# HandBrake/HandBrake

Measured on AMD Instinct MI355X. Metric: filtered frames/sec, 1080p YUV420p NLMeans+decomb chain, higher is better.
Workload: dtype u8 (f32 NLMeans weights, 16-bit fixed-point scaler as zimg, sharpen mix = the reference's f64 expression, as one f32 multiply where init proves that equal); 1 GPU; BASELINE configs[3]: decomb(31, EEDI2 bob) -> nlmeans medium -> cropscale lanczos 1920x1080 -> 3840x2160 -> lapsharp, 1080i YUV420P 8-bit in, inputs resident in HBM; input=1920x1080, output=3840x2160, streams_per_gpu=1, content=interlaced, stream_frames=48, stage_streams=2, parallelism=1 GPU(s) x 1 independent stream(s), device=AMD Radeon Graphics (gfx950:sramecc+:xnack-, 256 CUs)

## Files before the change

### handbrake_amd/csrc/eedi2.hip

```cpp
#include "eedi2_common.h"
#include "eedi2_vote.h"
#include "eedi2_dirmap_vote.h"
#include "eedi2_dense.h"
#include "eedi2_engine.h"
#include "eedi2_mask_cells.h"
#include "eedi2_corner.h"

#include <atomic>
#include <algorithm>

namespace {

constexpr int PEAK = 255, NEUTRAL = 128;
constexpr int EEDI_MAX_FIELDS = EEDI_MAX_BATCH;
constexpr size_t GUARD = 32768;

__constant__ uint8_t c_limlut[33] = { 6, 6, 7, 7, 8, 8, 9, 9, 9, 10, 10, 11, 11, 12, 12, 12, 12, 12, 12, 12,
                                      12, 12, 12, 12, 12, 12, 12, 12, 12, 12, 12, 255, 255 };

constexpr int LIM_N = 33, LIM_PAD = 40;
__device__ __forceinline__ void lim_fill(uint8_t *tab, int tid)
{
    if (tid < LIM_N) tab[tid] = c_limlut[tid];
}
// ... 377 lines not shown
        const uint8_t *mc = Q.a + (size_t)y * pitch;
        if (mc[x] == PEAK && (mc[x - 1] == PEAK || mc[x + 1] == PEAK))
            list[atomicAdd(count, 1)] = (uint32_t)x | ((uint32_t)y << 14) | ((uint32_t)pl << 28);
    }
}

__global__ __launch_bounds__(256) void k_calc_dir_work(P3 P, const uint32_t *__restrict__ list,
                                                       const int *__restrict__ count, int maxd, int nt13, int nt19)
{
    const int gid = blockIdx.x * blockDim.x + threadIdx.x;
    if (gid >= *count) return;
    const uint32_t e = list[gid];
    const int x = e & 0x3fff, y = (e >> 14) & 0x3fff, pl = e >> 28;
    const PL Q = plane_ptrs(P, pl, 0);
    const int pitch = P.pitch[pl], width = P.width[pl], height = P.height[pl];
    const uint8_t *mc = Q.a + (size_t)y * pitch;
    const uint8_t *mp = mc - pitch, *mn = mc + pitch;
    const uint8_t *sc = Q.b + (size_t)y * pitch;
    const uint8_t *sp = sc - pitch, *sn = sc + pitch, *s2p = sp - pitch, *s2n = sn + pitch;
    const int maxdt = pl == 0 ? maxd : (maxd >> 1);
    const int startu = max(-x + 1, -maxdt), stopu = min(width - 2 - x, maxdt);
    const int vert = iabs((int)sc[x] - (int)sn[x]) + iabs((int)sc[x] - (int)sp[x]);
    int minb = min(nt13, vert * 6), mina = min(nt19, vert * 9);
    int minc = mina, mind = minb, mine = minb;
    int dira = -5000, dirb = -5000, dirc = -5000, dird = -5000, dire = -5000;
    for (int u = startu; u <= stopu; u++)
    {
        if (!(y == 1 || mp[x - 1 + u] == PEAK || mp[x + u] == PEAK || mp[x + 1 + u] == PEAK)) continue;
        if (!(y == height - 2 || mn[x - 1 - u] == PEAK || mn[x - u] == PEAK || mn[x + 1 - u] == PEAK)) continue;
        const int diffsn = sad3(sc, x, sn, x - u);
        const int diffsp = sad3(sc, x, sp, x + u);
        const int diffps = sad3(sp, x, sc, x - u);
        const int diffns = sad3(sn, x, sc, x + u);
        const int diff = diffsn + diffsp + diffps + diffns;
        int diffd = diffsp + diffns, diffe = diffsn + diffps;
        if (diff < minb) { dirb = u; minb = diff; }
        if (y > 1)
        {
            const int diff2pp = sad3(s2p, x, sp, x - u);
            const int diffp2p = sad3(sp, x, s2p, x + u);
            const int diffa = diff + diff2pp + diffp2p;
            diffd += diffp2p;
            diffe += diff2pp;
            if (diffa < mina) { dira = u; mina = diffa; }
        }
        if (y < height - 2)
        {
            const int diff2nn = sad3(s2n, x, sn, x + u);
            const int diffn2n = sad3(sn, x, s2n, x - u);
            const int diffc = diff + diff2nn + diffn2n;
            diffd += diff2nn;
            diffe += diffn2n;
            if (diffc < minc) { dirc = u; minc = diffc; }
        }
        if (diffd < mind) { dird = u; mind = diffd; }
        if (diffe < mine) { dire = u; mine = diffe; }
    }
    int order[5], k = 0;
    if (dira != -5000) order[k++] = dira;
    if (dirb != -5000) order[k++] = dirb;
    if (dirc != -5000) order[k++] = dirc;
    if (dird != -5000) order[k++] = dird;
    if (dire != -5000) order[k++] = dire;
    int out = NEUTRAL;
    if (k > 1)
    {
        const int mid = sorted_mid(order, k);
        const int tlim = max((int)c_limlut[iabs(mid)] >> 2, 2);
        int sum = 0, cnt = 0;
        for (int i = 0; i < k; i++)
            if (iabs(order[i] - mid) <= tlim) { cnt++; sum += order[i]; }
        if (cnt > 1) out = (NEUTRAL + ((int)((float)sum / (float)cnt) * 4)) & 0xff;
    }
    Q.c[(size_t)y * pitch + x] = (uint8_t)out;
}

#ifdef HBHIP_DEV_STATS
__device__ unsigned long long g_cd_stats[24];
#define CD_STAT(i, v) atomicAdd(&g_cd_stats[i], (unsigned long long)(v))
#else
#define CD_STAT(i, v) ((void)0)
#endif
constexpr int CD_W = 256, CD_HALO = 32, CD_LW = CD_W + 2 * CD_HALO;



__device__ __forceinline__ int calc_dir_vote(int ta, int tb, int tc, int td, int te)
{
    constexpr int BIG = 1 << 20;
    int v0 = ta ? ta - 32 : BIG, v1 = tb ? tb - 32 : BIG, v2 = tc ? tc - 32 : BIG, v3 = td ? td - 32 : BIG, v4 = te ? te - 32 : BIG;
    const int k = (ta != 0) + (tb != 0) + (tc != 0) + (td != 0) + (te != 0);
#define CD_CX(a, b) { const int lo_ = min(a, b), hi_ = max(a, b); a = lo_; b = hi_; }
    CD_CX(v0, v1) CD_CX(v3, v4) CD_CX(v2, v4) CD_CX(v2, v3) CD_CX(v0, v3) CD_CX(v0, v2) CD_CX(v1, v4) CD_CX(v1, v3) CD_CX(v1, v2)
#undef CD_CX
    int out = NEUTRAL;
    if (k > 1)
    {
        const int lo = k == 2 ? v0 : (k == 5 ? v2 : v1);
        const int hi = k >= 4 ? v2 : v1;
        const int mid = (lo + hi + 1) >> 1;
        static_assert(CD_HALO - 2 <= 30, "the closed form of limlut covers entries 0..30");
        const int tlim = iabs(mid) >= 13 ? 3 : 2;
        int sum = 0, cnt = 0;
        if (iabs(v0 - mid) <= tlim) { cnt++; sum += v0; }
        if (iabs(v1 - mid) <= tlim) { cnt++; sum += v1; }
        if (iabs(v2 - mid) <= tlim) { cnt++; sum += v2; }
        if (iabs(v3 - mid) <= tlim) { cnt++; sum += v3; }
        if (iabs(v4 - mid) <= tlim) { cnt++; sum += v4; }
        if (cnt > 1) out = (NEUTRAL + ((int)((float)sum / (float)cnt) * 4)) & 0xff;
    }
    return out;
}

template <bool EDGE, typename PASS>
__device__ __forceinline__ int calc_dir_search(const uint32_t *tr, PASS pass, int maxdt, bool first, bool last, int nt13, int nt19)
{
    const uint32_t F2p = tr[0], Fp = tr[CD_LW], Fc = tr[2 * CD_LW], Fn = tr[3 * CD_LW], F2n = tr[4 * CD_LW];
    const int ctr = (int)((Fc >> 8) & 0xff);
    const int vert = iabs(ctr - (int)((Fn >> 8) & 0xff)) + iabs(ctr - (int)((Fp >> 8) & 0xff));
    uint32_t kb = (uint32_t)min(nt13, vert * 6) << 16, ka = (uint32_t)min(nt19, vert * 9) << 16;
    uint32_t kc = ka, kd = kb, ke = kb;
    typedef __attribute__((address_space(3))) const uint32_t *lds_u32;
    uint32_t ap0 = (uint32_t)(uintptr_t)(lds_u32)(tr - maxdt), am0 = (uint32_t)(uintptr_t)(lds_u32)(tr + maxdt);
    uint32_t tag0 = (uint32_t)(32 - maxdt);
    asm volatile("" : "+v"(ap0), "+v"(am0), "+s"(tag0));
#define SADH(a, b, acc) __builtin_amdgcn_sad_hi_u8((a), (b), (acc))
    while (pass)
    {
        const int jj = sizeof(PASS) == 8 ? __ffsll((unsigned long long)pass) - 1 : __ffs((unsigned int)pass) - 1;
        pass &= pass - (PASS)1;
        const uint32_t tag = (uint32_t)jj + tag0;
        const lds_u32 tp = (lds_u32)(uintptr_t)(ap0 + 4u * (uint32_t)jj), tm = (lds_u32)(uintptr_t)(am0 - 4u * (uint32_t)jj);
        const uint32_t e1 = SADH(Fp, tm[2 * CD_LW], SADH(Fc, tm[3 * CD_LW], 0u));
        const uint32_t d1 = SADH(Fn, tp[2 * CD_LW], SADH(Fc, tp[1 * CD_LW], tag));
        const uint32_t diff = e1 + d1;
        uint32_t diffd = d1, diffe = e1;
        kb = min(kb, diff);
        if (!EDGE || !first)
        {
            const uint32_t diff2pp = SADH(F2p, tm[1 * CD_LW], tag);
            const uint32_t diffp2p = SADH(Fp, tp[0 * CD_LW], 0u);
            diffd += diffp2p;
            diffe += diff2pp;
            ka = min(ka, diff + diff2pp + diffp2p);
        }
        else
            diffe += tag;
        if (!EDGE || !last)
        {
            const uint32_t diff2nn = SADH(F2n, tp[3 * CD_LW], 0u);
            const uint32_t diffn2n = SADH(Fn, tm[4 * CD_LW], 0u);
            diffd += diff2nn;
            diffe += diffn2n;
            kc = min(kc, diff + diff2nn + diffn2n);
        }
        kd = min(kd, diffd);
        ke = min(ke, diffe);
    }
#undef SADH
    return calc_dir_vote((int)((ka & 0xffffu) >> 1), (int)(kb & 0xffffu), (int)(kc & 0xffffu), (int)(kd & 0xffffu), (int)(ke & 0xffffu));
}

template <int R, bool PRED>
__device__ __forceinline__ void calc_dir_dense(const uint32_t *tr, int maxdt, const uint32_t (&up)[R], const uint32_t (&dn)[R],
                                               int nt13, int nt19, uint32_t (&ka)[R], uint32_t (&kb)[R], uint32_t (&kc)[R],
                                               uint32_t (&kd)[R], uint32_t (&ke)[R])
{
    constexpr int NS = R + 4, NE = R + 3;
#define SADH(a, b, acc) __builtin_amdgcn_sad_hi_u8((a), (b), (acc))
    uint32_t T[NS];
#pragma unroll
    for (int r = 0; r < NS; r++) T[r] = tr[r * CD_LW];
#pragma unroll
    for (int j = 0; j < R; j++)
    {
        const int ctr = (int)((T[j + 2] >> 8) & 0xff);
        const int vert = iabs(ctr - (int)((T[j + 3] >> 8) & 0xff)) + iabs(ctr - (int)((T[j + 1] >> 8) & 0xff));
        kb[j] = (uint32_t)min(nt13, vert * 6) << 16; ka[j] = (uint32_t)min(nt19, vert * 9) << 16;
        kc[j] = ka[j]; kd[j] = kb[j]; ke[j] = kb[j];
    }
    {
        CdRun<R, PRED> run;
#pragma unroll
        for (int r = 0; r < NE; r++)
        {
            const uint32_t Pv = SADH(T[r], T[r + 1], 32u);
            run.push(r, Pv, Pv);
            if (r >= 3)
            {
                const int j = r - 3;
                const uint32_t X = PRED ? (up[j] << 30) & 0x40000000u : 0u;
                uint32_t ca, cb, cc, cd, ce;
                run.cands(j, X, ca, cb, cc, cd, ce);
                ka[j] = min(ka[j], ca); kb[j] = min(kb[j], cb); kc[j] = min(kc[j], cc); kd[j] = min(kd[j], cd); ke[j] = min(ke[j], ce);
                CD_FENCE_KEYS(j);
            }
        }
    }
    for (int d = 1; d <= maxdt; d++)
    {
        const uint32_t *tp = tr + d, *tm = tr - d;
        const uint32_t t1 = 32u + (uint32_t)d, t2 = 32u - (uint32_t)d, sh = 30u - (uint32_t)d;
        CdRun<R, PRED> pos, neg;
        uint32_t Pl0 = tp[0], Mi0 = tm[0], Pl1 = tp[CD_LW], Mi1 = tm[CD_LW];
#pragma unroll
        for (int r = 0; r < NE; r++)
        {
            uint32_t Pl2 = 0, Mi2 = 0;
            if (r + 2 < NS) { Pl2 = tp[(r + 2) * CD_LW]; Mi2 = tm[(r + 2) * CD_LW]; }
            pos.push(r, SADH(T[r], Mi1, t1), SADH(Pl0, T[r + 1], t1));
            neg.push(r, SADH(T[r], Pl1, t2), SADH(Mi0, T[r + 1], t2));
            Pl0 = Pl1; Mi0 = Mi1; Pl1 = Pl2; Mi1 = Mi2;
            if (r >= 3)
            {
                const int j = r - 3;
                const uint32_t X1 = PRED ? (up[j] << sh) & 0x40000000u : 0u, X2 = PRED ? (dn[j] << sh) & 0x40000000u : 0u;
                uint32_t ca, cb, cc, cd, ce, na, nb, nc, nd, ne;
                pos.cands(j, X1, ca, cb, cc, cd, ce);
                neg.cands(j, X2, na, nb, nc, nd, ne);
                ka[j] = min(ka[j], min(ca, na)); kb[j] = min(kb[j], min(cb, nb)); kc[j] = min(kc[j], min(cc, nc));
                kd[j] = min(kd[j], min(cd, nd)); ke[j] = min(ke[j], min(ce, ne));
                CD_FENCE_KEYS(j);
            }
        }
    }
#undef SADH
}

template <int N, bool PRED, int RD, int J0>
__device__ __forceinline__ void calc_dir_dense_vote(const uint32_t *tr, int maxdt, const uint32_t (&up)[RD], const uint32_t (&dn)[RD],
                                                    uint32_t act, int nt13, int nt19, uint8_t *out)
{
    uint32_t u[N], v[N], ka[N], kb[N], kc[N], kd[N], ke[N];
#pragma unroll
    for (int j = 0; j < N; j++) { u[j] = up[J0 + j]; v[j] = dn[J0 + j]; }
    calc_dir_dense<N, PRED>(tr + J0 * CD_LW, maxdt, u, v, nt13, nt19, ka, kb, kc, kd, ke);
#pragma unroll
    for (int j = 0; j < N; j++)
        if ((act >> (J0 + j)) & 1u)
            out[(J0 + j) * CD_W] = (uint8_t)calc_dir_vote((int)((ka[j] & 0xffffu) / 6u), (int)((kb[j] & 0xffffu) >> 2), (int)((kc[j] & 0xffffu) / 6u),
                                                          (int)((kd[j] & 0xffffu) >> 2), (int)((ke[j] & 0xffffu) >> 2));
}

#ifndef CD_WAVES_ATTR
#define CD_WAVES_ATTR
#endif
template <int R>
__global__ __launch_bounds__(CD_W) CD_WAVES_ATTR void k_calc_dir_rows(P3 P, int maxd, int nt13, int nt19, int dense_min, uint32_t padv)
{
    constexpr int NS = R + 4, NM = R + 2, RW = CD_LW / 4, RQ = CD_LW / 16;
    __shared__ __attribute__((aligned(16))) uint8_t s_band[NS + NM][CD_LW];
    __shared__ __attribute__((aligned(16))) uint32_t s_tri[NS][CD_LW];
    __shared__ uint64_t s_bits[NM][8];
    __shared__ uint16_t s_list[R * CD_W];
    __shared__ __attribute__((aligned(16))) uint8_t s_out[R][CD_W];
    __shared__ int s_count;
    FIELD_PLANE(P);
    const int pitch = P.pitch[pl], width = P.width[pl], height = P.height[pl];
    const int x0 = blockIdx.x * CD_W, y0 = blockIdx.y * R;
    if (y0 >= height || x0 >= pitch) return;
    const int tid = threadIdx.x, lane = tid & 63;
    if (maskless)
    {
#pragma unroll
        for (int jr = 0; jr < R; jr += CD_W / 64)
        {
            const int j = jr + (tid >> 6), y = y0 + j, xb = x0 + 4 * lane;
            if (j < R && y < height && xb < pitch) *reinterpret_cast<uint32_t *>(Q.c + (size_t)y * pitch + xb) = pad_bytes(0xffffffffu, xb, width, padv);
        }
        return;
    }
    if (tid == 0) s_count = 0;
    if (tid < NM * 3) s_bits[tid / 3][5 + tid % 3] = 0;
    uint32_t *band = reinterpret_cast<uint32_t *>(&s_band[0][0]);
    {
        const uint8_t *sb = Q.b + x0 - CD_HALO, *mb = Q.a + x0 - CD_HALO;
        for (int i = tid; i < (NS + NM) * RQ; i += CD_W)
        {
            const int r = i / RQ, c16 = i - r * RQ;
            const uint8_t *src = r < NS ? sb + (ptrdiff_t)min(y0 - 2 + r, height + 1) * pitch
                                        : mb + (ptrdiff_t)min(y0 - 1 + (r - NS), height) * pitch;
            reinterpret_cast<uint4 *>(band)[i] = reinterpret_cast<const uint4 *>(src)[c16];
        }
    }
    __syncthreads();
#pragma unroll
    for (int jr = 0; jr < R; jr += CD_W / 64)
    {
        const int j = jr + (tid >> 6), y = y0 + j, xb = x0 + 4 * lane;
        if (R % (CD_W / 64) != 0 && j >= R) break;
        const uint32_t *mrow = band + (NS + j + 1) * RW + CD_HALO / 4 + lane;
        const uint32_t prev = mrow[-1], cur = mrow[0], next = mrow[1];
        auto eq255 = [](uint32_t v) { return (((v & 0x7f7f7f7fu) + 0x01010101u) & v) & 0x80808080u; };
        uint32_t act = eq255(cur) & (eq255(__builtin_amdgcn_alignbyte(cur, prev, 3)) | eq255(__builtin_amdgcn_alignbyte(next, cur, 1)));
        if (y < 1 || y >= height - 1) act = 0;
#pragma unroll
        for (int k = 0; k < 4; k++)
            if (xb + k < 1 || xb + k >= width - 1) act &= ~(0x80u << (8 * k));
        reinterpret_cast<uint32_t *>(&s_out[j][0])[lane] = 0xffffffffu;
        int total = 0, before = 0;
#pragma unroll
        for (int k = 0; k < 4; k++)
        {
            const uint64_t bal = __ballot((act >> (8 * k + 7)) & 1u);
            before += (int)__builtin_amdgcn_mbcnt_hi((uint32_t)(bal >> 32), __builtin_amdgcn_mbcnt_lo((uint32_t)bal, 0u));
            total += __popcll(bal);
        }
        int base = 0;
        if (lane == 0 && total) base = atomicAdd(&s_count, total);
        base = __builtin_amdgcn_readfirstlane(base) + before;
#pragma unroll
        for (int k = 0; k < 4; k++)
            if ((act >> (8 * k + 7)) & 1u) s_list[base++] = (uint16_t)((j << 8) | (4 * lane + k));
    }
    __syncthreads();
    const int count = s_count;
    const int maxdt = pl == 0 ? maxd : (maxd >> 1);
    const int len = 2 * maxdt + 1;
    const uint64_t lenmask = (1ull << len) - 1ull;
    const bool edge = y0 <= 1 || y0 + R - 1 >= height - 2;
    const bool dense = R >= 4 && !edge && count >= dense_min;
    if (count)
    {
// ... 1930 lines not shown
```

### handbrake_amd/csrc/eedi2_16.hip

```cpp
#include "eedi2_common.h"
#include "eedi2_engine.h"
#include "eedi2_mask_cells.h"
#include "eedi2_corner.h"
#include <algorithm>

namespace {

constexpr size_t GUARD16 = 32768;

struct K16
{
    int peak, neutral, shift;
    int limlut[33];
};

struct Q3
{
    uint16_t *a[3], *b[3], *c[3];
    uint16_t *d[3], *e[3], *f[3], *g[3];
    int pitch[3], width[3], height[3];
    size_t   fstride;
    uint32_t tffbits;
    const uint32_t *pflags;
    uint32_t pepoch;
};

struct QL { uint16_t *a, *b, *c; };
__device__ __forceinline__ QL plane_ptrs16(const Q3 &P, int pl, size_t off)
{
    return QL{ P.a[pl] + off, P.b[pl] + off, P.c[pl] + off };
}
#define FIELD16(P)                                                           \
    const int fld = (int)blockIdx.z / 3, pl = (int)blockIdx.z - 3 * fld;     \
    const int tff = (int)(((P).tffbits >> fld) & 1u);                        \
    const QL Q = plane_ptrs16((P), pl, (size_t)fld * (P).fstride);           \
    const bool maskless = (P).pflags[blockIdx.z] != (P).pepoch;              \
    (void)tff; (void)maskless

#define XY16(P)                                                              \
    FIELD16(P);                                                              \
    const int x = blockIdx.x * blockDim.x + threadIdx.x;                     \
    const int y = blockIdx.y * blockDim.y + threadIdx.y;                     \
    const int pitch = (P).pitch[pl], width = (P).width[pl], height = (P).height[pl]; \
    (void)width; (void)height; (void)pitch

__device__ __forceinline__ int sad3w(const uint16_t *a, int ai, const uint16_t *b, int bi)
{
    return iabs((int)a[ai - 1] - (int)b[bi - 1]) + iabs((int)a[ai] - (int)b[bi]) + iabs((int)a[ai + 1] - (int)b[bi + 1]);
}

#ifndef QM_TILE_W
#define QM_TILE_W 128
#endif
#ifndef QM_THREADS
#define QM_THREADS 512
#endif
using QM = EediMaskGeo<QM_TILE_W, 16, 2, QM_THREADS>;

struct MaskSrc16 { const uint16_t *frame[EEDI_MAX_BATCH][3]; int sp[3]; };

template <bool CHAIN>
__device__ __forceinline__ void qmask_tile(const Q3 &P, const MaskSrc16 &S, const K16 &k, const MaskChain &C, int fld, int pl, int bx, int by,
                                           int mth, int vth, int lth, int erode_thr, int dilate_thr,
                                           uint16_t (*s_src)[QM::LP + 8], uint32_t (*s_a)[QM::DP], uint32_t (*s_b)[QM::DP])
{
    const int pitch = P.pitch[pl], width = P.width[pl], height = P.height[pl];
    const int x0 = bx * QM::W, y0 = by * QM::H;
    const bool upper = y0 + QM::H + QM::OY <= height / 2;
    const size_t foff = (size_t)fld * P.fstride;
    const uint16_t *oldm = fld == 0 ? P.b[pl] : P.c[pl] + foff - P.fstride;
    const uint16_t *frame = S.frame[fld][pl];
    const int start_line = (int)(((P.tffbits >> fld) & 1u) ^ 1u);
    uint16_t *srcp = P.a[pl] + foff, *newm = P.c[pl] + foff;
    const int t = threadIdx.x, fx = x0 - QM::OX, fy = y0 - QM::OY;
    const int peak = k.peak, sh = k.shift;

    for (int i = t; i < QM::LR * QM::DW; i += QM::T)
    {
        const int r = i / QM::DW, c4 = i - r * QM::DW;
        const int y = fy + r, x = fx + 4 * c4;
        uint2 sv = make_uint2(0u, 0u);
        if (y >= 0 && y < height && x >= 0 && x < pitch)
        {
            if (x < width)
            {
                sv = *reinterpret_cast<const uint2 *>(frame + (size_t)(start_line + 2 * y) * S.sp[pl] + x);
// ... 206 lines not shown
            if (!(y == 1 || mp[x - 1 + u] == peak || mp[x + u] == peak || mp[x + 1 + u] == peak)) continue;
            if (!(y == height - 2 || mn[x - 1 - u] == peak || mn[x - u] == peak || mn[x + 1 - u] == peak)) continue;
            const int diffsn = sad3w(sc, x, sn, x - u);
            const int diffsp = sad3w(sc, x, sp, x + u);
            const int diffps = sad3w(sp, x, sc, x - u);
            const int diffns = sad3w(sn, x, sc, x + u);
            const int diff = diffsn + diffsp + diffps + diffns;
            int diffd = diffsp + diffns, diffe = diffsn + diffps;
            if (diff < minb) { dirb = u; minb = diff; }
            if (y > 1)
            {
                const int diff2pp = sad3w(s2p, x, sp, x - u);
                const int diffp2p = sad3w(sp, x, s2p, x + u);
                const int diffa = diff + diff2pp + diffp2p;
                diffd += diffp2p;
                diffe += diff2pp;
                if (diffa < mina) { dira = u; mina = diffa; }
            }
            if (y < height - 2)
            {
                const int diff2nn = sad3w(s2n, x, sn, x + u);
                const int diffn2n = sad3w(sn, x, s2n, x - u);
                const int diffc = diff + diff2nn + diffn2n;
                diffd += diff2nn;
                diffe += diffn2n;
                if (diffc < minc) { dirc = u; minc = diffc; }
            }
            if (diffd < mind) { dird = u; mind = diffd; }
            if (diffe < mine) { dire = u; mine = diffe; }
        }
        int order[5], n = 0;
        if (dira != -5000) order[n++] = dira;
        if (dirb != -5000) order[n++] = dirb;
        if (dirc != -5000) order[n++] = dirc;
        if (dird != -5000) order[n++] = dird;
        if (dire != -5000) order[n++] = dire;
        out = k.neutral;
        if (n > 1)
        {
            const int mid = sorted_mid(order, n);
            const int tlim = max(k.limlut[iabs(mid)] >> 2, 2);
            int sum = 0, count = 0;
            for (int i = 0; i < n; i++)
                if (iabs(order[i] - mid) <= tlim) { count++; sum += order[i]; }
            if (count > 1) out = (uint16_t)(k.neutral + ((int)((float)sum / (float)count) << (2 + k.shift)));
        }
    }
    Q.c[(size_t)y * pitch + x] = (uint16_t)out;
}

constexpr int QW = 256, QHALO = 32, QLW = QW + 2 * QHALO;

__device__ __forceinline__ uint32_t sad3q(uint2 a, uint2 b, uint32_t acc)
{
    return __builtin_amdgcn_sad_u16(a.x, b.x, __builtin_amdgcn_sad_u16(a.y, b.y, acc));
}

__device__ __forceinline__ int calc_dir_vote16(int ta, int tb, int tc, int td, int te, const int *limlut, int neutral, int shift)
{
    constexpr int BIG = 1 << 20;
    int v0 = ta ? ta - 32 : BIG, v1 = tb ? tb - 32 : BIG, v2 = tc ? tc - 32 : BIG, v3 = td ? td - 32 : BIG, v4 = te ? te - 32 : BIG;
    const int n = (ta != 0) + (tb != 0) + (tc != 0) + (td != 0) + (te != 0);
#define Q_CX(a, b) { const int lo_ = min(a, b), hi_ = max(a, b); a = lo_; b = hi_; }
    Q_CX(v0, v1) Q_CX(v3, v4) Q_CX(v2, v4) Q_CX(v2, v3) Q_CX(v0, v3) Q_CX(v0, v2) Q_CX(v1, v4) Q_CX(v1, v3) Q_CX(v1, v2)
#undef Q_CX
    int out = neutral;
    if (n > 1)
    {
        const int lo = n == 2 ? v0 : (n == 5 ? v2 : v1);
        const int hi = n >= 4 ? v2 : v1;
        const int mid = (lo + hi + 1) >> 1;
        const int tlim = max(limlut[iabs(mid)] >> 2, 2);
        int sum = 0, cnt = 0;
        if (iabs(v0 - mid) <= tlim) { cnt++; sum += v0; }
        if (iabs(v1 - mid) <= tlim) { cnt++; sum += v1; }
        if (iabs(v2 - mid) <= tlim) { cnt++; sum += v2; }
        if (iabs(v3 - mid) <= tlim) { cnt++; sum += v3; }
        if (iabs(v4 - mid) <= tlim) { cnt++; sum += v4; }
        if (cnt > 1) out = (uint16_t)(neutral + ((int)((float)sum / (float)cnt) << (2 + shift)));
    }
    return out;
}

template <int R, bool PRED>
__device__ __forceinline__ void calc_dir_dense16(const uint2 *tr, int maxdt, const uint32_t (&up)[R], const uint32_t (&dn)[R],
                                                 int nt13, int nt19, uint32_t (&ka)[R], uint32_t (&kb)[R], uint32_t (&kc)[R],
                                                 uint32_t (&kd)[R], uint32_t (&ke)[R])
{
    constexpr int NS = R + 4, NE = R + 3;
    uint2 T[NS];
#pragma unroll
    for (int r = 0; r < NS; r++) T[r] = tr[r * QLW];
#pragma unroll
    for (int j = 0; j < R; j++)
    {
        const int ctr = (int)(T[j + 2].x >> 16);
        const int vert = iabs(ctr - (int)(T[j + 3].x >> 16)) + iabs(ctr - (int)(T[j + 1].x >> 16));
        kb[j] = (uint32_t)min(nt13, vert * 6) << 9; ka[j] = (uint32_t)min(nt19, vert * 9) << 9;
        kc[j] = ka[j]; kd[j] = kb[j]; ke[j] = kb[j];
    }
    auto term = [](uint2 a, uint2 b, uint32_t tag) { return (sad3q(a, b, 0u) << 9) + tag; };
    auto sums = [&](const uint32_t (&Pv)[NE], const uint32_t (&Qv)[NE], const uint32_t (&X)[R], uint32_t (&ca)[R], uint32_t (&cb)[R],
                    uint32_t (&cc)[R], uint32_t (&cd)[R], uint32_t (&ce)[R]) {
        uint32_t S[NE], P2[NE - 1], Q2[NE - 1];
#pragma unroll
        for (int r = 0; r < NE; r++) S[r] = Pv[r] + Qv[r];
#pragma unroll
        for (int r = 0; r < NE - 1; r++) { P2[r] = Pv[r] + Pv[r + 1]; Q2[r] = Qv[r] + Qv[r + 1]; }
        if (PRED)
        {
#pragma unroll
            for (int j = 0; j < R; j++)
            {
                cb[j] = S[j + 1] + S[j + 2] + X[j]; ca[j] = cb[j] + S[j]; cc[j] = cb[j] + S[j + 3];
                ce[j] = P2[j] + P2[j + 2] + X[j];   cd[j] = Q2[j] + Q2[j + 2] + X[j];
            }
        }
        else
        {
            uint32_t S2[NE - 1], S3[NE - 2];
#pragma unroll
            for (int r = 0; r < NE - 1; r++) S2[r] = S[r] + S[r + 1];
#pragma unroll
            for (int r = 0; r < NE - 2; r++) S3[r] = S2[r] + S[r + 2];
#pragma unroll
            for (int j = 0; j < R; j++)
            {
                cb[j] = S2[j + 1]; ca[j] = S3[j]; cc[j] = S3[j + 1];
                ce[j] = P2[j] + P2[j + 2]; cd[j] = Q2[j] + Q2[j + 2];
            }
        }
    };
    uint32_t X1[R], X2[R];
#pragma unroll
    for (int j = 0; j < R; j++) { X1[j] = 0; X2[j] = 0; }
    {
        uint32_t Pv[NE], ca[R], cb[R], cc[R], cd[R], ce[R];
#pragma unroll
        for (int r = 0; r < NE; r++) Pv[r] = term(T[r], T[r + 1], 32u);
        if (PRED)
        {
#pragma unroll
            for (int j = 0; j < R; j++) X1[j] = (up[j] << 30) & 0x40000000u;
        }
        sums(Pv, Pv, X1, ca, cb, cc, cd, ce);
#pragma unroll
        for (int j = 0; j < R; j++)
        {
            ka[j] = min(ka[j], ca[j]); kb[j] = min(kb[j], cb[j]); kc[j] = min(kc[j], cc[j]);
            kd[j] = min(kd[j], cd[j]); ke[j] = min(ke[j], ce[j]);
        }
    }
    for (int d = 1; d <= maxdt; d++)
    {
        const uint2 *tp = tr + d, *tm = tr - d;
        uint2 Pl[NS], Mi[NS];
#pragma unroll
        for (int r = 0; r < NS; r++) { Pl[r] = tp[r * QLW]; Mi[r] = tm[r * QLW]; }
        const uint32_t t1 = 32u + (uint32_t)d, t2 = 32u - (uint32_t)d;
        uint32_t P1[NE], Q1[NE], Pn[NE], Qn[NE];
#pragma unroll
        for (int r = 0; r < NE; r++)
        {
            P1[r] = term(T[r], Mi[r + 1], t1); Q1[r] = term(Pl[r], T[r + 1], t1);
            Pn[r] = term(T[r], Pl[r + 1], t2); Qn[r] = term(Mi[r], T[r + 1], t2);
        }
        if (PRED)
        {
            const uint32_t sh = 30u - (uint32_t)d;
#pragma unroll
            for (int j = 0; j < R; j++) { X1[j] = (up[j] << sh) & 0x40000000u; X2[j] = (dn[j] << sh) & 0x40000000u; }
        }
        uint32_t ca[R], cb[R], cc[R], cd[R], ce[R], na[R], nb[R], nc[R], nd[R], ne[R];
        sums(P1, Q1, X1, ca, cb, cc, cd, ce);
        sums(Pn, Qn, X2, na, nb, nc, nd, ne);
#pragma unroll
        for (int j = 0; j < R; j++)
        {
            ka[j] = min(ka[j], min(ca[j], na[j])); kb[j] = min(kb[j], min(cb[j], nb[j])); kc[j] = min(kc[j], min(cc[j], nc[j]));
            kd[j] = min(kd[j], min(cd[j], nd[j])); ke[j] = min(ke[j], min(ce[j], ne[j]));
        }
    }
}

template <bool EDGE>
__device__ __forceinline__ int calc_dir_search16(const uint2 *tr, uint64_t pass, int maxdt, bool first, bool last, int nt13, int nt19,
                                                 const int *limlut, int neutral, int shift)
{
    const uint2 F2p = tr[0], Fp = tr[QLW], Fc = tr[2 * QLW], Fn = tr[3 * QLW], F2n = tr[4 * QLW];
    const int ctr = (int)(Fc.x >> 16);
    const int vert = iabs(ctr - (int)(Fn.x >> 16)) + iabs(ctr - (int)(Fp.x >> 16));
    uint32_t kb = (uint32_t)min(nt13, vert * 6) << 6, ka = (uint32_t)min(nt19, vert * 9) << 6;
    uint32_t kc = ka, kd = kb, ke = kb;
    while (pass)
    {
        const int jj = __ffsll((unsigned long long)pass) - 1;
        pass &= pass - 1ull;
        const int u = jj - maxdt;
        const uint32_t ub = (uint32_t)(u + 32);
        const uint2 *tp = tr + u, *tm = tr - u;
        const uint32_t e1 = sad3q(Fp, tm[2 * QLW], sad3q(Fc, tm[3 * QLW], 0u));
        const uint32_t d1 = sad3q(Fn, tp[2 * QLW], sad3q(Fc, tp[1 * QLW], 0u));
        const uint32_t diff = e1 + d1;
        uint32_t diffd = d1, diffe = e1;
        kb = min(kb, (diff << 6) | ub);
        if (!EDGE || !first)
        {
            const uint32_t diff2pp = sad3q(F2p, tm[1 * QLW], 0u);
            const uint32_t diffp2p = sad3q(Fp, tp[0 * QLW], 0u);
            diffd += diffp2p;
            diffe += diff2pp;
            ka = min(ka, ((diff + diff2pp + diffp2p) << 6) | ub);
        }
        if (!EDGE || !last)
        {
            const uint32_t diff2nn = sad3q(F2n, tp[3 * QLW], 0u);
            const uint32_t diffn2n = sad3q(Fn, tm[4 * QLW], 0u);
            diffd += diff2nn;
            diffe += diffn2n;
            kc = min(kc, ((diff + diff2nn + diffn2n) << 6) | ub);
        }
        kd = min(kd, (diffd << 6) | ub);
        ke = min(ke, (diffe << 6) | ub);
    }
    return calc_dir_vote16((int)(ka & 63u), (int)(kb & 63u), (int)(kc & 63u), (int)(kd & 63u), (int)(ke & 63u), limlut, neutral, shift);
}

__device__ __forceinline__ uint32_t pad_pair16(uint32_t v, int X, int width, int padv)
{
    if (X >= width) return (uint32_t)padv * 0x00010001u;
    if (X + 1 >= width) return (v & 0xffffu) | ((uint32_t)padv << 16);
    return v;
}


template <int R>
__global__ __launch_bounds__(QW) void q_calc_dir_rows(Q3 P, K16 k, int maxd, int nt, int dense_min, int padv)
{
    constexpr int NS = R + 4, NM = R + 2, RWD = QLW / 2;
    __shared__ __attribute__((aligned(16))) uint16_t s_band[NS + NM][QLW];
    __shared__ uint2    s_tri[NS][QLW];
    __shared__ uint64_t s_pk[NM][8];
    __shared__ uint16_t s_list[R * QW];
    __shared__ __attribute__((aligned(16))) uint16_t s_out[R][QW];
    __shared__ int s_lim[33];
    __shared__ int s_count;
    FIELD16(P);
    const int pitch = P.pitch[pl], width = P.width[pl], height = P.height[pl];
    const int x0 = blockIdx.x * QW, y0 = blockIdx.y * R;
    if (y0 >= height || x0 >= pitch) return;
    const int tid = threadIdx.x, lane = tid & 63;
    const int peak = k.peak;
    if (maskless)
    {
        const uint32_t pk2 = (uint32_t)peak | ((uint32_t)peak << 16);
        for (int i = tid; i < R * (QW / 2); i += QW)
        {
            const int j = i / (QW / 2), c2 = i - j * (QW / 2), y = y0 + j, xb = x0 + 2 * c2;
            if (y < height && xb < pitch) *reinterpret_cast<uint32_t *>(Q.c + (size_t)y * pitch + xb) = pad_pair16(pk2, xb, width, padv);
        }
        return;
    }
    if (tid == 0) s_count = 0;
// ... 9 lines not shown
                                         : mb + (ptrdiff_t)min(y0 - 1 + (r - NS), height) * pitch;
            band[i] = reinterpret_cast<const uint32_t *>(src)[c2];
        }
    }
    __syncthreads();
    for (int rnd = 0; rnd < 2; rnd++)
    {
        if (rnd == 1 && tid >= 64) break;
        const int i = tid + rnd * QW;
        if (i < QLW - 2)
        {
            const int q = i >> 1;
            const uint32_t sh = (uint32_t)(i & 1) * 2u;
#pragma unroll
            for (int r = 0; r < NS; r++)
            {
                const uint32_t d0 = band[r * RWD + q], d1 = band[r * RWD + q + 1];
                s_tri[r][i] = make_uint2(__builtin_amdgcn_alignbyte(d1, d0, sh), (d1 >> (8u * sh)) & 0xffffu);
            }
        }
#pragma unroll
        for (int m = 0; m < NM; m++)
        {
            const uint64_t w = __ballot(i < QLW && s_band[NS + m][i < QLW ? i : 0] == peak);
            if (lane == 0 && i < QLW) s_pk[m][i >> 6] = w;
        }
    }
#pragma unroll
    for (int j = 0; j < R; j++)
    {
        const int y = y0 + j, x = x0 + tid;
        const uint16_t *m = &s_band[NS + j + 1][tid + QHALO];
        const bool act = y >= 1 && y < height - 1 && x >= 1 && x < width - 1 && m[0] == peak && (m[-1] == peak || m[1] == peak);
        s_out[j][tid] = (uint16_t)peak;
        const uint64_t bal = __ballot(act);
        int base = 0;
        if (lane == 0 && bal) base = atomicAdd(&s_count, __popcll(bal));
        base = __builtin_amdgcn_readfirstlane(base);
        if (act) s_list[base + (int)__builtin_amdgcn_mbcnt_hi((uint32_t)(bal >> 32), __builtin_amdgcn_mbcnt_lo((uint32_t)bal, 0u))] = (uint16_t)((j << 8) | tid);
    }
    __syncthreads();
    const int count = s_count;
    const int nt13 = (uint16_t)((nt << k.shift) * 13), nt19 = (uint16_t)((nt << k.shift) * 19);
    const int maxdt = pl == 0 ? maxd : (maxd >> 1);
    const int len = 2 * maxdt + 1;
    const uint64_t lenmask = (1ull << len) - 1ull;
    const bool edge = y0 <= 1 || y0 + R - 1 >= height - 2;
    if (R >= 4 && !edge && count >= dense_min)
    {
        constexpr int RD = R >= 4 ? R : 1;
        const int lx = tid, px = x0 + lx, b = lx + QHALO - 1;
        const int startu = max(-px + 1, -maxdt), stopu = min(width - 2 - px, maxdt);
        uint64_t range = 0;
        if (stopu >= startu)
        {
            const int nb = stopu - startu + 1;
            range = (nb >= 64 ? ~0ull : ((1ull << nb) - 1ull)) << (startu + maxdt);
        }
        uint64_t win[RD + 2];
#pragma unroll
        for (int m = 0; m < RD + 2; m++) win[m] = calc_dir_window(s_pk[m], b - maxdt, lenmask);
        uint32_t up[RD], dn[RD], act = 0, inactive = 0;
#pragma unroll
        for (int j = 0; j < RD; j++)
        {
            const uint16_t *m = &s_band[NS + j + 1][tid + QHALO];
            const bool a = px >= 1 && px < width - 1 && m[0] == peak && (m[-1] == peak || m[1] == peak);
            const uint64_t pass = a ? range & win[j] & (__brevll(win[j + 2]) >> (64 - len)) : 0ull;
            const uint64_t npass = ~pass;
            up[j] = (uint32_t)(npass >> maxdt);
            dn[j] = __brev((uint32_t)npass << (31 - maxdt));
            act |= (uint32_t)a << j;
            inactive |= (up[j] | dn[j]) & ((2u << maxdt) - 1u);
        }
        if (__any(act != 0))
        {
            uint32_t ka[RD], kb[RD], kc[RD], kd[RD], ke[RD];
            const uint2 *tr = &s_tri[0][b];
            if (__all(inactive == 0)) calc_dir_dense16<RD, false>(tr, maxdt, up, dn, nt13, nt19, ka, kb, kc, kd, ke);
            else                      calc_dir_dense16<RD, true>(tr, maxdt, up, dn, nt13, nt19, ka, kb, kc, kd, ke);
#pragma unroll
            for (int j = 0; j < RD; j++)
                if ((act >> j) & 1u)
                    s_out[j][lx] = (uint16_t)calc_dir_vote16((int)((ka[j] & 511u) / 6u), (int)((kb[j] & 511u) >> 2), (int)((kc[j] & 511u) / 6u),
                                                             (int)((kd[j] & 511u) >> 2), (int)((ke[j] & 511u) >> 2), s_lim, k.neutral, k.shift);
        }
        __syncthreads();
    }
    else if (count)
    {
        for (int p = tid; p < count; p += QW)
        {
            const uint32_t id = s_list[p];
            const int j = (int)(id >> 8), lx = (int)(id & 255u), y = y0 + j, px = x0 + lx, b = lx + QHALO - 1;
            const int startu = max(-px + 1, -maxdt), stopu = min(width - 2 - px, maxdt);
            auto any3 = [&](const uint64_t *bits) {
                const int start = b - maxdt, wq = start >> 6, sh = start & 63;
                const uint64_t lo = bits[wq], hi = bits[wq + 1];
                const uint64_t w = sh ? (lo >> sh) | (hi << (64 - sh)) : lo;
                return (w | (w >> 1) | (w >> 2)) & lenmask;
            };
            uint64_t pass = 0;
            if (stopu >= startu)
            {
                const int nb = stopu - startu + 1;
                pass = (nb >= 64 ? ~0ull : ((1ull << nb) - 1ull)) << (startu + maxdt);
                if (y != 1)          pass &= any3(s_pk[j]);
                if (y != height - 2) pass &= __brevll(any3(s_pk[j + 2])) >> (64 - len);
            }
            const uint2 *tr = &s_tri[j][b];
            const int out = edge ? calc_dir_search16<true>(tr, pass, maxdt, y == 1, y == height - 2, nt13, nt19, s_lim, k.neutral, k.shift)
                                 : calc_dir_search16<false>(tr, pass, maxdt, false, false, nt13, nt19, s_lim, k.neutral, k.shift);
            s_out[j][lx] = (uint16_t)out;
        }
        __syncthreads();
    }
#pragma unroll
    for (int i = tid; i < R * (QW / 2); i += QW)
    {
        const int j = i / (QW / 2), c2 = i - j * (QW / 2), y = y0 + j, xb = x0 + 2 * c2;
        if (y < height && xb < pitch)
            *reinterpret_cast<uint32_t *>(Q.c + (size_t)y * pitch + xb) = pad_pair16(reinterpret_cast<const uint32_t *>(&s_out[j][0])[c2], xb, width, padv);
    }
}

constexpr int ABSENT16 = 1 << 20;

__device__ __forceinline__ int mid9q(int &v0, int &v1, int &v2, int &v3, int &v4, int &v5, int &v6, int &v7, int &v8, int n)
{
    cswap(v0, v3); cswap(v1, v7); cswap(v2, v5); cswap(v4, v8);
    cswap(v0, v7); cswap(v2, v4); cswap(v3, v8); cswap(v5, v6);
    cswap(v0, v2); cswap(v1, v3); cswap(v4, v5); cswap(v7, v8);
    cswap(v1, v4); cswap(v3, v6); cswap(v5, v7);
    cswap(v0, v1); cswap(v2, v4); cswap(v3, v5); cswap(v6, v8);
    cswap(v2, v3); cswap(v4, v5); cswap(v6, v7);
    cswap(v1, v2); cswap(v3, v4); cswap(v5, v6);
    const int lo = n <= 4 ? v1 : (n <= 6 ? v2 : (n <= 8 ? v3 : v4));
    const int hi = n <= 5 ? v2 : (n <= 7 ? v3 : v4);
    return (n & 1) ? hi : (lo + hi + 1) >> 1;
}

__device__ __forceinline__ void vote1q(int v, int mid, int lim, int &sum, int &cnt)
{
    const bool in = iabs(v - mid) <= lim;
    cnt += in;
    sum += in ? v : 0;
}

__device__ __forceinline__ int dir_map_px16(int u0, int u1, int u2, int c0, int c1, int c2, int n0, int n1, int n2,
                                            bool up_ok, bool dn_ok, int expand, int peak, int neutral, int sh2, const int *limlut)
{
    const bool h0 = up_ok && u0 != peak, h1 = up_ok && u1 != peak, h2 = up_ok && u2 != peak;
    const bool h3 = c0 != peak, h4 = !expand && c1 != peak, h5 = c2 != peak;
    const bool h6 = dn_ok && n0 != peak, h7 = dn_ok && n1 != peak, h8 = dn_ok && n2 != peak;
    const int u = h0 + h1 + h2 + h3 + h4 + h5 + h6 + h7 + h8;
    if (u < (expand ? 5 : 4)) return expand ? c1 : peak;
    int v0 = h0 ? u0 : ABSENT16, v1 = h1 ? u1 : ABSENT16, v2 = h2 ? u2 : ABSENT16;
    int v3 = h3 ? c0 : ABSENT16, v4 = h4 ? c1 : ABSENT16, v5 = h5 ? c2 : ABSENT16;
    int v6 = h6 ? n0 : ABSENT16, v7 = h7 ? n1 : ABSENT16, v8 = h8 ? n2 : ABSENT16;
    const int mid = mid9q(v0, v1, v2, v3, v4, v5, v6, v7, v8, u);
    const int lim = limlut[iabs(mid - neutral) >> sh2];
    int sum = 0, count = 0;
    vote1q(v0, mid, lim, sum, count); vote1q(v1, mid, lim, sum, count); vote1q(v2, mid, lim, sum, count);
    vote1q(v3, mid, lim, sum, count); vote1q(v4, mid, lim, sum, count); vote1q(v5, mid, lim, sum, count);
    vote1q(v6, mid, lim, sum, count); vote1q(v7, mid, lim, sum, count); vote1q(v8, mid, lim, sum, count);
    const int val = (int)(((float)(sum + mid) / (float)(count + 1)) + 0.5f);
    if (expand) return count >= 5 ? val : c1;
// ... 1468 lines not shown
```

### handbrake_amd/csrc/eedi2_dense.h

```cpp
#pragma once
#include <hip/hip_runtime.h>
#include <cstdint>

template <int R, bool PRED>
struct CdRun
{
    static constexpr int NE = R + 3;
    uint32_t P[NE], Q[NE], S[NE], P2[NE], Q2[NE], S2[NE], S3[NE];
    __device__ __forceinline__ void push(int r, uint32_t p, uint32_t q)
    {
        P[r] = p; Q[r] = q; S[r] = p + q;
        if (r >= 1) { P2[r - 1] = P[r - 1] + p; Q2[r - 1] = Q[r - 1] + q; }
        if (!PRED && r >= 1) S2[r - 1] = S[r - 1] + S[r];
        if (!PRED && r >= 2) S3[r - 2] = S2[r - 2] + S[r];
    }
    __device__ __forceinline__ void cands(int j, uint32_t X, uint32_t &ca, uint32_t &cb, uint32_t &cc, uint32_t &cd, uint32_t &ce) const
    {
        if (PRED)
        {
            cb = S[j + 1] + S[j + 2] + X; ca = cb + S[j]; cc = cb + S[j + 3];
            ce = P2[j] + P2[j + 2] + X;   cd = Q2[j] + Q2[j + 2] + X;
        }
        else
        {
            cb = S2[j + 1]; ca = S3[j]; cc = S3[j + 1];
            ce = P2[j] + P2[j + 2]; cd = Q2[j] + Q2[j + 2];
        }
    }
};

#define CD_FENCE_KEYS(j) asm volatile("" : "+v"(ka[j]), "+v"(kb[j]), "+v"(kc[j]), "+v"(kd[j]), "+v"(ke[j]))
```

Baseline: 10030 output frames/s.

## Restructure EEDI2 dense direction sums to share partial SADs across keys

Rewrites the dense calc_dir kernels, 8- and 16-bit, to accumulate SADs in place instead of adding them afterwards. The S term is now built by chaining the second SAD onto the first, so keys a, b and c carry doubled weight and the final divisors are adjusted to match. The e key is derived as a total minus the d key rather than summed separately. In the non-predicated path, keys a and c are tracked as one running minimum over shared window sums and resolved once at the end, which cuts per-step min operations and register state. This leans on tag-bit headroom, asserted at compile time, and the arithmetic identities must hold exactly or the output could change.

Result: no change. 10110 output frames/s (median of 6 runs) (+0.8%).

```diff
diff --git a/handbrake_amd/csrc/eedi2.hip b/handbrake_amd/csrc/eedi2.hip
--- a/handbrake_amd/csrc/eedi2.hip
+++ b/handbrake_amd/csrc/eedi2.hip
@@ -483,6 +483,7 @@
 #define CD_STAT(i, v) ((void)0)
 #endif
 constexpr int CD_W = 256, CD_HALO = 32, CD_LW = CD_W + 2 * CD_HALO;
+static_assert(CD_HALO - 2 == CD_MAX_DIST, "the dense keys' tag bound (eedi2_dense.h) is for the widest search the halo takes");
 
 
 
@@ -570,31 +571,36 @@
     constexpr int NS = R + 4, NE = R + 3;
 #define SADH(a, b, acc) __builtin_amdgcn_sad_hi_u8((a), (b), (acc))
     uint32_t T[NS];
+    [[maybe_unused]] uint32_t M[R + 1];
 #pragma unroll
     for (int r = 0; r < NS; r++) T[r] = tr[r * CD_LW];
+    auto vert = [&](int j) {
+        const int ctr = (int)((T[j + 2] >> 8) & 0xff);
+        return iabs(ctr - (int)((T[j + 3] >> 8) & 0xff)) + iabs(ctr - (int)((T[j + 1] >> 8) & 0xff));
+    };
 #pragma unroll
     for (int j = 0; j < R; j++)
     {
-        const int ctr = (int)((T[j + 2] >> 8) & 0xff);
-        const int vert = iabs(ctr - (int)((T[j + 3] >> 8) & 0xff)) + iabs(ctr - (int)((T[j + 1] >> 8) & 0xff));
-        kb[j] = (uint32_t)min(nt13, vert * 6) << 16; ka[j] = (uint32_t)min(nt19, vert * 9) << 16;
-        kc[j] = ka[j]; kd[j] = kb[j]; ke[j] = kb[j];
+        kb[j] = (uint32_t)min(nt13, vert(j) * 6) << 16; kd[j] = kb[j]; ke[j] = kb[j];
+        if (PRED) { ka[j] = (uint32_t)min(nt19, vert(j) * 9) << 16; kc[j] = ka[j]; }
     }
     {
         CdRun<R, PRED> run;
 #pragma unroll
         for (int r = 0; r < NE; r++)
         {
-            const uint32_t Pv = SADH(T[r], T[r + 1], 32u);
-            run.push(r, Pv, Pv);
+            const uint32_t Qv = SADH(T[r], T[r + 1], 32u);
+            run.push(r, Qv, SADH(T[r], T[r + 1], Qv));
+            if constexpr (!PRED) { if (r >= 2) M[r - 2] = run.S3[r - 2]; }
             if (r >= 3)
             {
                 const int j = r - 3;
                 const uint32_t X = PRED ? (up[j] << 30) & 0x40000000u : 0u;
                 uint32_t ca, cb, cc, cd, ce;
-                run.cands(j, X, ca, cb, cc, cd, ce);
-                ka[j] = min(ka[j], ca); kb[j] = min(kb[j], cb); kc[j] = min(kc[j], cc); kd[j] = min(kd[j], cd); ke[j] = min(ke[j], ce);
-                CD_FENCE_KEYS(j);
+                run.cands(j, 128u, X, ca, cb, cc, cd, ce);
+                kb[j] = min(kb[j], cb); kd[j] = min(kd[j], cd); ke[j] = min(ke[j], ce);
+                if constexpr (PRED) { ka[j] = min(ka[j], ca); kc[j] = min(kc[j], cc); CD_FENCE_KEYS(j); }
+                else CD_FENCE_KEYS_M(j);
             }
         }
     }
@@ -602,6 +608,8 @@
     {
         const uint32_t *tp = tr + d, *tm = tr - d;
         const uint32_t t1 = 32u + (uint32_t)d, t2 = 32u - (uint32_t)d, sh = 30u - (uint32_t)d;
+        uint32_t q1 = 4u * t1, q2 = 4u * t2;
+        asm("" : "+s"(q1), "+s"(q2));
         CdRun<R, PRED> pos, neg;
         uint32_t Pl0 = tp[0], Mi0 = tm[0], Pl1 = tp[CD_LW], Mi1 = tm[CD_LW];
 #pragma unroll
@@ -609,20 +617,35 @@
         {
             uint32_t Pl2 = 0, Mi2 = 0;
             if (r + 2 < NS) { Pl2 = tp[(r + 2) * CD_LW]; Mi2 = tm[(r + 2) * CD_LW]; }
-            pos.push(r, SADH(T[r], Mi1, t1), SADH(Pl0, T[r + 1], t1));
-            neg.push(r, SADH(T[r], Pl1, t2), SADH(Mi0, T[r + 1], t2));
+            const uint32_t Qp = SADH(Pl0, T[r + 1], t1), Qn = SADH(Mi0, T[r + 1], t2);
+            pos.push(r, Qp, SADH(T[r], Mi1, Qp));
+            neg.push(r, Qn, SADH(T[r], Pl1, Qn));
             Pl0 = Pl1; Mi0 = Mi1; Pl1 = Pl2; Mi1 = Mi2;
+            if constexpr (!PRED) { if (r >= 2) M[r - 2] = min(M[r - 2], min(pos.S3[r - 2], neg.S3[r - 2])); }
             if (r >= 3)
             {
                 const int j = r - 3;
                 const uint32_t X1 = PRED ? (up[j] << sh) & 0x40000000u : 0u, X2 = PRED ? (dn[j] << sh) & 0x40000000u : 0u;
                 uint32_t ca, cb, cc, cd, ce, na, nb, nc, nd, ne;
-                pos.cands(j, X1, ca, cb, cc, cd, ce);
-                neg.cands(j, X2, na, nb, nc, nd, ne);
-                ka[j] = min(ka[j], min(ca, na)); kb[j] = min(kb[j], min(cb, nb)); kc[j] = min(kc[j], min(cc, nc));
-                kd[j] = min(kd[j], min(cd, nd)); ke[j] = min(ke[j], min(ce, ne));
-                CD_FENCE_KEYS(j);
-            }
+                pos.cands(j, q1, X1, ca, cb, cc, cd, ce);
+                neg.cands(j, q2, X2, na, nb, nc, nd, ne);
+                kb[j] = min(kb[j], min(cb, nb)); kd[j] = min(kd[j], min(cd, nd)); ke[j] = min(ke[j], min(ce, ne));
+                if constexpr (PRED)
+                {
+                    ka[j] = min(ka[j], min(ca, na)); kc[j] = min(kc[j], min(cc, nc));
+                    CD_FENCE_KEYS(j);
+                }
+                else CD_FENCE_KEYS_M(j);
+            }
+        }
+    }
+    if constexpr (!PRED)
+    {
+#pragma unroll
+        for (int j = 0; j < R; j++)
+        {
+            const uint32_t init = (uint32_t)min(nt19, vert(j) * 9) << 16;
+            ka[j] = min(init, M[j]); kc[j] = min(init, M[j + 1]);
         }
     }
 #undef SADH
@@ -639,7 +662,7 @@
 #pragma unroll
     for (int j = 0; j < N; j++)
         if ((act >> (J0 + j)) & 1u)
-            out[(J0 + j) * CD_W] = (uint8_t)calc_dir_vote((int)((ka[j] & 0xffffu) / 6u), (int)((kb[j] & 0xffffu) >> 2), (int)((kc[j] & 0xffffu) / 6u),
+            out[(J0 + j) * CD_W] = (uint8_t)calc_dir_vote((int)((ka[j] & 0xffffu) / 3u), (int)((kb[j] & 0xffffu) >> 1), (int)((kc[j] & 0xffffu) / 3u),
                                                           (int)((kd[j] & 0xffffu) >> 2), (int)((ke[j] & 0xffffu) >> 2));
 }
 
diff --git a/handbrake_amd/csrc/eedi2_16.hip b/handbrake_amd/csrc/eedi2_16.hip
--- a/handbrake_amd/csrc/eedi2_16.hip
+++ b/handbrake_amd/csrc/eedi2_16.hip
@@ -2,6 +2,7 @@
 #include "eedi2_engine.h"
 #include "eedi2_mask_cells.h"
 #include "eedi2_corner.h"
+#include "eedi2_dense.h"
 #include <algorithm>
 
 namespace {
@@ -374,6 +375,7 @@
     return out;
 }
 
+static_assert(QHALO - 2 == CD_MAX_DIST, "the dense keys' tag bound (eedi2_dense.h) is for the widest search the halo takes");
 template <int R, bool PRED>
 __device__ __forceinline__ void calc_dir_dense16(const uint2 *tr, int maxdt, const uint32_t (&up)[R], const uint32_t (&dn)[R],
                                                  int nt13, int nt19, uint32_t (&ka)[R], uint32_t (&kb)[R], uint32_t (&kc)[R],
@@ -381,45 +383,59 @@
 {
     constexpr int NS = R + 4, NE = R + 3;
     uint2 T[NS];
+    [[maybe_unused]] uint32_t M[R + 1];
 #pragma unroll
     for (int r = 0; r < NS; r++) T[r] = tr[r * QLW];
+    auto vert = [&](int j) {
+        const int ctr = (int)(T[j + 2].x >> 16);
+        return iabs(ctr - (int)(T[j + 3].x >> 16)) + iabs(ctr - (int)(T[j + 1].x >> 16));
+    };
 #pragma unroll
     for (int j = 0; j < R; j++)
     {
-        const int ctr = (int)(T[j + 2].x >> 16);
-        const int vert = iabs(ctr - (int)(T[j + 3].x >> 16)) + iabs(ctr - (int)(T[j + 1].x >> 16));
-        kb[j] = (uint32_t)min(nt13, vert * 6) << 9; ka[j] = (uint32_t)min(nt19, vert * 9) << 9;
-        kc[j] = ka[j]; kd[j] = kb[j]; ke[j] = kb[j];
-    }
-    auto term = [](uint2 a, uint2 b, uint32_t tag) { return (sad3q(a, b, 0u) << 9) + tag; };
-    auto sums = [&](const uint32_t (&Pv)[NE], const uint32_t (&Qv)[NE], const uint32_t (&X)[R], uint32_t (&ca)[R], uint32_t (&cb)[R],
-                    uint32_t (&cc)[R], uint32_t (&cd)[R], uint32_t (&ce)[R]) {
-        uint32_t S[NE], P2[NE - 1], Q2[NE - 1];
-#pragma unroll
-        for (int r = 0; r < NE; r++) S[r] = Pv[r] + Qv[r];
-#pragma unroll
-        for (int r = 0; r < NE - 1; r++) { P2[r] = Pv[r] + Pv[r + 1]; Q2[r] = Qv[r] + Qv[r + 1]; }
+        kb[j] = (uint32_t)min(nt13, vert(j) * 6) << 9; kd[j] = kb[j]; ke[j] = kb[j];
+        if (PRED) { ka[j] = (uint32_t)min(nt19, vert(j) * 9) << 9; kc[j] = ka[j]; }
+    }
+    auto terms = [](uint2 own, uint2 other, uint2 qa, uint2 qb, uint32_t tag, uint32_t &Qv, uint32_t &Sv) {
+        const uint32_t q = sad3q(qa, qb, 0u);
+        Qv = cd_opaque((q << 9) + tag); Sv = cd_opaque((sad3q(own, other, q) << 9) + tag);
+    };
+    auto sums = [&](const uint32_t (&Qv)[NE], const uint32_t (&Sv)[NE], uint32_t t4, const uint32_t (&X)[R], uint32_t (&ca)[R],
+                    uint32_t (&cb)[R], uint32_t (&cc)[R], uint32_t (&cd)[R], uint32_t (&ce)[R], uint32_t (&S3)[R + 1]) {
+        uint32_t QQ[NE];
+        auto shared = [](int r) { return r >= 2 && r <= R - 1; };
+#pragma unroll
+        for (int r = 0; r < NE - 1; r++)
+            if (shared(r)) QQ[r] = cd_opaque(Qv[r] + Qv[r + 1]);
+        auto q4 = [&](int j) {
+            if (shared(j) && shared(j + 2)) return QQ[j] + QQ[j + 2];
+            if (shared(j)) return QQ[j] + Qv[j + 2] + Qv[j + 3];
+            if (shared(j + 2)) return Qv[j] + Qv[j + 1] + QQ[j + 2];
+            return Qv[j] + Qv[j + 1] + (Qv[j + 2] + Qv[j + 3]);
+        };
         if (PRED)
         {
 #pragma unroll
             for (int j = 0; j < R; j++)
             {
-                cb[j] = S[j + 1] + S[j + 2] + X[j]; ca[j] = cb[j] + S[j]; cc[j] = cb[j] + S[j + 3];
-                ce[j] = P2[j] + P2[j + 2] + X[j];   cd[j] = Q2[j] + Q2[j + 2] + X[j];
+                const uint32_t d4 = cd_opaque(q4(j));
+                cb[j] = Sv[j + 1] + Sv[j + 2] + X[j]; ca[j] = cb[j] + Sv[j]; cc[j] = cb[j] + Sv[j + 3];
+                ce[j] = (ca[j] + Sv[j + 3] + t4) - d4; cd[j] = d4 + X[j];
             }
         }
         else
         {
-            uint32_t S2[NE - 1], S3[NE - 2];
-#pragma unroll
-            for (int r = 0; r < NE - 1; r++) S2[r] = S[r] + S[r + 1];
-#pragma unroll
-            for (int r = 0; r < NE - 2; r++) S3[r] = S2[r] + S[r + 2];
+            uint32_t SS[NE];
+#pragma unroll
+            for (int r = 1; r <= R; r++) SS[r] = Sv[r] + Sv[r + 1];
+            S3[0] = Sv[0] + SS[1];
+#pragma unroll
+            for (int r = 1; r <= R; r++) S3[r] = SS[r] + Sv[r + 2];
 #pragma unroll
             for (int j = 0; j < R; j++)
             {
-                cb[j] = S2[j + 1]; ca[j] = S3[j]; cc[j] = S3[j + 1];
-                ce[j] = P2[j] + P2[j + 2]; cd[j] = Q2[j] + Q2[j + 2];
+                cb[j] = SS[j + 1];
+                cd[j] = cd_opaque(q4(j)); ce[j] = (S3[j] + Sv[j + 3] + t4) - cd[j];
             }
         }
     };
@@ -427,20 +443,25 @@
 #pragma unroll
     for (int j = 0; j < R; j++) { X1[j] = 0; X2[j] = 0; }
     {
-        uint32_t Pv[NE], ca[R], cb[R], cc[R], cd[R], ce[R];
-#pragma unroll
-        for (int r = 0; r < NE; r++) Pv[r] = term(T[r], T[r + 1], 32u);
+        uint32_t Qv[NE], Sv[NE], ca[R], cb[R], cc[R], cd[R], ce[R], S3[R + 1];
+#pragma unroll
+        for (int r = 0; r < NE; r++) terms(T[r], T[r + 1], T[r], T[r + 1], 32u, Qv[r], Sv[r]);
         if (PRED)
         {
 #pragma unroll
             for (int j = 0; j < R; j++) X1[j] = (up[j] << 30) & 0x40000000u;
         }
-        sums(Pv, Pv, X1, ca, cb, cc, cd, ce);
+        sums(Qv, Sv, 128u, X1, ca, cb, cc, cd, ce, S3);
 #pragma unroll
         for (int j = 0; j < R; j++)
         {
-            ka[j] = min(ka[j], ca[j]); kb[j] = min(kb[j], cb[j]); kc[j] = min(kc[j], cc[j]);
-            kd[j] = min(kd[j], cd[j]); ke[j] = min(ke[j], ce[j]);
+            kb[j] = min(kb[j], cb[j]); kd[j] = min(kd[j], cd[j]); ke[j] = min(ke[j], ce[j]);
+            if (PRED) { ka[j] = min(ka[j], ca[j]); kc[j] = min(kc[j], cc[j]); }
+        }
+        if (!PRED)
+        {
+#pragma unroll
+            for (int r = 0; r <= R; r++) M[r] = S3[r];
         }
     }
     for (int d = 1; d <= maxdt; d++)
@@ -450,12 +471,14 @@
 #pragma unroll
         for (int r = 0; r < NS; r++) { Pl[r] = tp[r * QLW]; Mi[r] = tm[r * QLW]; }
         const uint32_t t1 = 32u + (uint32_t)d, t2 = 32u - (uint32_t)d;
-        uint32_t P1[NE], Q1[NE], Pn[NE], Qn[NE];
+        uint32_t q1 = 4u * t1, q2 = 4u * t2;
+        asm("" : "+s"(q1), "+s"(q2));
+        uint32_t Q1[NE], S1[NE], Qn[NE], Sn[NE];
 #pragma unroll
         for (int r = 0; r < NE; r++)
         {
-            P1[r] = term(T[r], Mi[r + 1], t1); Q1[r] = term(Pl[r], T[r + 1], t1);
-            Pn[r] = term(T[r], Pl[r + 1], t2); Qn[r] = term(Mi[r], T[r + 1], t2);
+            terms(T[r], Mi[r + 1], Pl[r], T[r + 1], t1, Q1[r], S1[r]);
+            terms(T[r], Pl[r + 1], Mi[r], T[r + 1], t2, Qn[r], Sn[r]);
         }
         if (PRED)
         {
@@ -463,14 +486,28 @@
 #pragma unroll
             for (int j = 0; j < R; j++) { X1[j] = (up[j] << sh) & 0x40000000u; X2[j] = (dn[j] << sh) & 0x40000000u; }
         }
-        uint32_t ca[R], cb[R], cc[R], cd[R], ce[R], na[R], nb[R], nc[R], nd[R], ne[R];
-        sums(P1, Q1, X1, ca, cb, cc, cd, ce);
-        sums(Pn, Qn, X2, na, nb, nc, nd, ne);
+        uint32_t ca[R], cb[R], cc[R], cd[R], ce[R], na[R], nb[R], nc[R], nd[R], ne[R], S3p[R + 1], S3n[R + 1];
+        sums(Q1, S1, q1, X1, ca, cb, cc, cd, ce, S3p);
+        sums(Qn, Sn, q2, X2, na, nb, nc, nd, ne, S3n);
 #pragma unroll
         for (int j = 0; j < R; j++)
         {
-            ka[j] = min(ka[j], min(ca[j], na[j])); kb[j] = min(kb[j], min(cb[j], nb[j])); kc[j] = min(kc[j], min(cc[j], nc[j]));
-            kd[j] = min(kd[j], min(cd[j], nd[j])); ke[j] = min(ke[j], min(ce[j], ne[j]));
+            kb[j] = min(kb[j], min(cb[j], nb[j])); kd[j] = min(kd[j], min(cd[j], nd[j])); ke[j] = min(ke[j], min(ce[j], ne[j]));
+            if (PRED) { ka[j] = min(ka[j], min(ca[j], na[j])); kc[j] = min(kc[j], min(cc[j], nc[j])); }
+        }
+        if (!PRED)
+        {
+#pragma unroll
+            for (int r = 0; r <= R; r++) M[r] = min(M[r], min(S3p[r], S3n[r]));
+        }
+    }
+    if (!PRED)
+    {
+#pragma unroll
+        for (int j = 0; j < R; j++)
+        {
+            const uint32_t init = (uint32_t)min(nt19, vert(j) * 9) << 9;
+            ka[j] = min(init, M[j]); kc[j] = min(init, M[j + 1]);
         }
     }
 }
@@ -646,7 +683,7 @@
 #pragma unroll
             for (int j = 0; j < RD; j++)
                 if ((act >> j) & 1u)
-                    s_out[j][lx] = (uint16_t)calc_dir_vote16((int)((ka[j] & 511u) / 6u), (int)((kb[j] & 511u) >> 2), (int)((kc[j] & 511u) / 6u),
+                    s_out[j][lx] = (uint16_t)calc_dir_vote16((int)((ka[j] & 511u) / 3u), (int)((kb[j] & 511u) >> 1), (int)((kc[j] & 511u) / 3u),
                                                              (int)((kd[j] & 511u) >> 2), (int)((ke[j] & 511u) >> 2), s_lim, k.neutral, k.shift);
         }
         __syncthreads();
diff --git a/handbrake_amd/csrc/eedi2_dense.h b/handbrake_amd/csrc/eedi2_dense.h
--- a/handbrake_amd/csrc/eedi2_dense.h
+++ b/handbrake_amd/csrc/eedi2_dense.h
@@ -1,32 +1,48 @@
 #pragma once
 #include <hip/hip_runtime.h>
 #include <cstdint>
+
+constexpr int CD_MAX_DIST = 30;
+static_assert(8 * (32 + CD_MAX_DIST) < (1 << 9), "eight tags of the widest step fit the 9 tag bits of the 16-bit keys (and the 16 of the 8-bit ones)");
+
+__device__ __forceinline__ uint32_t cd_opaque(uint32_t v) { asm("" : "+v"(v)); return v; }
 
 template <int R, bool PRED>
 struct CdRun
 {
     static constexpr int NE = R + 3;
-    uint32_t P[NE], Q[NE], S[NE], P2[NE], Q2[NE], S2[NE], S3[NE];
-    __device__ __forceinline__ void push(int r, uint32_t p, uint32_t q)
+    uint32_t Q[NE], S[NE], QQ[NE], SS[NE], S3[NE];
+    static constexpr bool shared(int r) { return r >= 2 && r <= R - 1; }
+    __device__ __forceinline__ void push(int r, uint32_t q, uint32_t s)
     {
-        P[r] = p; Q[r] = q; S[r] = p + q;
-        if (r >= 1) { P2[r - 1] = P[r - 1] + p; Q2[r - 1] = Q[r - 1] + q; }
-        if (!PRED && r >= 1) S2[r - 1] = S[r - 1] + S[r];
-        if (!PRED && r >= 2) S3[r - 2] = S2[r - 2] + S[r];
+        Q[r] = q; S[r] = s;
+        if (shared(r - 1)) QQ[r - 1] = cd_opaque(Q[r - 1] + q);
+        if (!PRED && r >= 2 && r <= R + 1) SS[r - 1] = S[r - 1] + s;
+        if (!PRED && r == 2) S3[0] = S[0] + SS[1];
+        if (!PRED && r >= 3) S3[r - 2] = SS[r - 2] + s;
     }
-    __device__ __forceinline__ void cands(int j, uint32_t X, uint32_t &ca, uint32_t &cb, uint32_t &cc, uint32_t &cd, uint32_t &ce) const
+    __device__ __forceinline__ uint32_t q4(int j) const
     {
+        if (shared(j) && shared(j + 2)) return QQ[j] + QQ[j + 2];
+        if (shared(j)) return QQ[j] + Q[j + 2] + Q[j + 3];
+        if (shared(j + 2)) return Q[j] + Q[j + 1] + QQ[j + 2];
+        return Q[j] + Q[j + 1] + (Q[j + 2] + Q[j + 3]);
+    }
+    __device__ __forceinline__ void cands(int j, uint32_t t4, uint32_t X, uint32_t &ca, uint32_t &cb, uint32_t &cc, uint32_t &cd, uint32_t &ce) const
+    {
+        const uint32_t d4 = cd_opaque(q4(j));
         if (PRED)
         {
             cb = S[j + 1] + S[j + 2] + X; ca = cb + S[j]; cc = cb + S[j + 3];
-            ce = P2[j] + P2[j + 2] + X;   cd = Q2[j] + Q2[j + 2] + X;
+            ce = (ca + S[j + 3] + t4) - d4; cd = d4 + X;
         }
         else
         {
-            cb = S2[j + 1]; ca = S3[j]; cc = S3[j + 1];
-            ce = P2[j] + P2[j + 2]; cd = Q2[j] + Q2[j + 2];
+            cb = SS[j + 1]; ca = S3[j]; cc = S3[j + 1];
+            cd = d4; ce = (S3[j] + S[j + 3] + t4) - d4;
         }
     }
 };
 
 #define CD_FENCE_KEYS(j) asm volatile("" : "+v"(ka[j]), "+v"(kb[j]), "+v"(kc[j]), "+v"(kd[j]), "+v"(ke[j]))
+#define CD_FENCE_KEYS_M(j) asm volatile("" : "+v"(M[(j) + 1]), "+v"(kb[j]), "+v"(kd[j]), "+v"(ke[j]))
```
